# AdrienCorenflos/aux-ssm-samplers

Hardware: AMD Instinct MI355X
Metric: Gibbs sweeps/sec (aux-Kalman, parallel-in-time scan) (higher is better)
Workload: dtype f64; 1 GPU; C2: linear-Gaussian SSM T=65536 d=4 p=8, aux-Kalman sweep, parallel scan; chains_per_gpu=256, parallelism=chains x1 (independent, no collective)

## Files before the change

aux_ssm_samplers_amd/csrc/api.hip:

```cpp
#include <cstdarg>
#include <cstdlib>
#include <cstring>

#include "ctx.h"
#include "rng.h"

namespace ax {

static thread_local std::string g_err;
void set_error(const char* fmt, ...) {
    char buf[1024];
    va_list ap;
    va_start(ap, fmt);
    vsnprintf(buf, sizeof buf, fmt, ap);
    va_end(ap);
    g_err = buf;
}

int ws_reserve(auxssm_ctx* h, size_t bytes) {
    h->ws_off = 0;
    if (bytes <= h->ws_bytes) return AUXSSM_OK;
    if (h->ws) {
        AX_HIP(hipStreamSynchronize(h->stream));
        AX_HIP(hipFree(h->ws));
// ... 620 lines not shown
    SampleArgs sa;
    sa.d = kd;
    sa.dx = D;
    sa.Fs = cv(model->Fs); sa.Qs = cv(model->Qs); sa.bs = cv(model->bs);
    sa.ms = msA; sa.Ps = PsA; sa.eps = epsA; sa.xs = xpA; sa.elem = nullptr;
    sa.lay = ScanLayout{1, 1, 1, 1, cm, C};
    sa.ps_shared = shared_mode ? 1 : 0;
    sa.ps_packed = ps_pack ? 1 : 0;
    if (gen) sa.eps_gen = 1, sa.gen_k0 = keys[2], sa.gen_k1 = keys[3];
    rc = se->sample(h, sa, parallel);
    if (rc) return rc;
    h->ws_off = mark;

    {
        SweepLogpdfArgs la;
        la.d = kd;
        la.dx = D; la.po = PO;
        la.m0 = cv(model->m0); la.P0 = cv(model->P0); la.Fs = cv(model->Fs); la.Qs = cv(model->Qs); la.bs = cv(model->bs);
        la.Hs = cv(model->Hs); la.Rs = cv(model->Rs); la.cs = cv(model->cs); la.ys = cv(*yobs);
        la.x = xA; la.xp = xpA; la.u = uA; la.delta = delta; la.nan_policy = nan_policy;
        la.u_fly = aux_fly ? 1 : 0; la.eps_aux = epsauxA; la.shd = sqrt(0.5 * delta); la.dptr = dptr;
        rc = sl->run(h, la, sums);
        if (rc) return rc;
        h->ws_off = mark;
    }
    const Acc* jp_prop = sums; const Acc* jp_rev = sums + C; const Acc* lt_prop = sums + 2 * C; const Acc* lt_rev = sums + 3 * C; const Acc* corr = sums + 4 * C;
    hipLaunchKernelGGL((k_accept<R>), dim3((C + 127) / 128), dim3(128), 0, h->stream, C, jp_prop, jp_rev, (const R*)ell, (const R*)ell, lt_prop, lt_rev,
                       corr, (const R*)u_acc, accepted, (R*)logs);
    if ((rc = launch_select<R>(h, C, T, D, (const int32_t*)accepted, xpA, xA, cm))) return rc;
    AX_HIP(hipGetLastError());
    return AUXSSM_OK;
}

template <typename R>
__global__ void k_fs_concat0(int C, int D, int PO, const R* __restrict__ xa, const R* __restrict__ xb, const int32_t* __restrict__ sel, const R* __restrict__ eps0, R shd,
                             const double* dptr, Arr yobs, R* __restrict__ u, R* __restrict__ ysc0) {
    if (dptr) shd = (R)dptr[1];
    const int P = D + PO;
    const int g = blockIdx.x * blockDim.x + threadIdx.x;
    if (g >= C * P) return;
    const int c = g % C, k = g / C;
    if (k < D) {
        const R* x = (sel && sel[c]) ? xb : xa;
        const R v = x[(long long)k * C + c] + shd * eps0[(long long)k * C + c];
        u[(long long)k * C + c] = v;
        ysc0[(long long)k * C + c] = v;
    } else {
        ysc0[(long long)k * C + c] = at<R>(yobs, 0, 0, 0)[k - D];
    }
}
template <typename R> __global__ void __launch_bounds__(256) k_fs_resolve(int C, const int32_t* __restrict__ sel, const R* __restrict__ xb, R* __restrict__ xa) {
    const int c = blockIdx.y * 256 + threadIdx.x;
    if (c >= C) return;
    const long long off = (long long)blockIdx.x * C + c;
    if (sel[c]) xa[off] = xb[off];
}
template <typename R>
__global__ void __launch_bounds__(256) k_fs_stats(int C, const int32_t* __restrict__ accepted, const int32_t* __restrict__ sel, const R* __restrict__ xa, const R* __restrict__ xb,
                                                   R* __restrict__ sq_jump, R* __restrict__ mean, R* __restrict__ sq_mean, long long iter) {
    const int c = blockIdx.y * 256 + threadIdx.x;
    if (c >= C) return;
    const long long off = (long long)blockIdx.x * C + c;
    const int s = sel[c], acc = accepted[c];
    const R xn = (s ? xb : xa)[off];
    const R xo = acc ? (s ? xa : xb)[off] : xn;
    const R it = (R)iter, dj = xn - xo;
    sq_jump[off] = fold_mean<R>(it, sq_jump[off], dj * dj);
    mean[off] = fold_mean<R>(it, mean[off], xn);
    sq_mean[off] = fold_mean<R>(it, sq_mean[off], xn * xn);
}
static const char* fused_refusal(const auxssm_ctx* h, const auxssm_dims* dims, const auxssm_lgssm* model, int parallel, int layout) {
    const int C = dims->C, T = dims->T, D = dims->dx, PO = dims->dy;
    if (layout != AUXSSM_LAYOUT_CHAIN_MINOR) return "the fused sweep takes the chain-minor layout";
    if (D > MAX_D || PO < 1 || PO > 4) return "the fused sweep is instantiated for dx <= 4, 1 <= dy <= 4";
    if (!parallel) return "the fused sweep is the parallel-in-time one";
    if (!h->share_model) return "AUXSSM_OPT_SHARE_MODEL is off";
    if (!(model->Fs.sc == 0 && model->Qs.sc == 0 && model->bs.sc == 0 && model->P0.sc == 0 && model->m0.sc == 0))
        return "the fused sweep needs chain-shared model parameters (chain stride 0)";
    if (C < 2 || (C % 2) != 0) return "the fused sweep pairs chains for its in-kernel draws: the chain count must be even";
    if (T < 64) return "the fused sweep needs T >= 64";
    return nullptr;
}
template <typename R>
static int sweep_lg_concat_fused(auxssm_ctx* h, int dtype, const auxssm_dims* dims, const auxssm_lgssm* model, const auxssm_arr* yobs, double delta, const double* dptr,
                                 const uint32_t* keys, int nan_policy, void* x, void* x_alt, int32_t* sel, void* u_acc, int32_t* accepted, void* logs) {
    const int C = dims->C, T = dims->T, D = dims->dx, PO = dims->dy, P = D + PO;
    const SweepLogpdfEntry* sl = sweep_logpdf_entry(dtype, D, PO);
    if (!sl || !sl->fused) {
        set_error("(dx=%d, dy=%d) has no fused sweep in this build", D, PO);
        return AUXSSM_ERR_UNSUPPORTED;
    }
    const KDims kd{C, T, 1};
    const size_t sR = sizeof(R), CT = (size_t)C * T;
    size_t need = 0;
    auto add = [&](size_t b) { need += b + 256; };
    add(CT * D * sR);
    add(CT * D * sR);
    add((size_t)T * (P * D + P * P + P + D * D) * sR);
    add(1024);
    add((size_t)C * (P + 3 * D) * sR + 1024);
    add(sl->fused_ws(h, kd));
    int rc = ws_reserve(h, need);
    if (rc) return rc;
    R* u = (R*)ws_take(h, CT * D * sR);
    R* inc = (R*)ws_take(h, CT * D * sR);
    R* ysc0 = (R*)ws_take(h, (size_t)C * P * sR);
    R* m0p = (R*)ws_take(h, (size_t)C * D * sR);
    R* eps0a = (R*)ws_take(h, (size_t)C * D * sR);
    R* eps0s = (R*)ws_take(h, (size_t)C * D * sR);
    if (!u || !inc || !ysc0 || !m0p || !eps0a || !eps0s) return AUXSSM_ERR_NOMEM;
    bool overlap = h->overlap_model_stage != 0 && !dptr;
    struct SweepEnd {
        auxssm_ctx* h;
        ~SweepEnd() { side_sweep_end(h); }
    } sweep_end{h};
    if (overlap) {
        const size_t need_side = sl->fused_ws(h, kd) + (size_t)(T + 64) * sR * ((size_t)P * D + (size_t)P * P + P + (size_t)D * D) + (4u << 20) +
                                 (size_t)(T + 2) * sR * (3 * (size_t)D * D + 2 * D + (size_t)PO * D + (size_t)PO * PO + 2 * PO);
        if ((rc = side_open(h, need_side))) return rc;
        overlap = h->side.open;
    }
    R *Hc, *Rc, *cc, *Ps;
    const bool tinv = model->Hs.st == 0 && model->Rs.st == 0 && model->cs.st == 0;
    const int Tm = tinv ? 1 : T;
    const int* memo = nullptr;
    struct MemoGuard {
        auxssm_ctx* h;
        int p = -1;
        bool ok = false;
        ~MemoGuard() { if (p >= 0 && !ok) h->side.memo_use[p] = -1; }
    } memo_guard{h};
    if (overlap) {
        SideScope sc(h);
        auxssm_ctx::SideStage& sd = h->side;
        const int p = sd.parity;
        MemoDesc md{};
        const auxssm_arr* srcs[9] = {&model->m0, &model->P0, &model->Fs, &model->Qs, &model->bs, &model->Hs, &model->Rs, &model->cs, yobs};
        const int recs[9] = {D, D * D, D * D, D * D, D, PO * D, PO * PO, PO, PO};
        const int nts[9] = {1, 1, T - 1, T - 1, T - 1, T, T, T, T};
        md.n = 9;
        md.off[0] = 0;
        bool plain = true;
        for (int q = 0; q < 9; ++q) {
// ... 10 lines not shown
            std::vector<unsigned char> key;
            auto put = [&](const void* v, size_t nb) { key.insert(key.end(), (const unsigned char*)v, (const unsigned char*)v + nb); };
            const int hdr[8] = {(int)sR, C, T, D, PO, nan_policy, 0, 0};
            put(hdr, sizeof(hdr));
            put(&delta, sizeof(delta));
            for (int q = 0; q < 9; ++q) put(srcs[q], sizeof(auxssm_arr));
            const bool chain_ok = sd.memo_use[p] == sd.uses[p] - 1 && sd.memo_key[p] == key;
            const unsigned gmemo = (unsigned)std::min<long long>(1024, (md.off[9] + 255) / 256);
            if (chain_ok) {
                hipLaunchKernelGGL(k_memo_set, dim3(1), dim3(1), 0, h->stream, rebuild, 0);
                hipLaunchKernelGGL((k_memo_check<R>), dim3(gmemo), dim3(256), 0, h->stream, md, (const R*)snap, rebuild);
            } else {
                hipLaunchKernelGGL(k_memo_set, dim3(1), dim3(1), 0, h->stream, rebuild, 1);
            }
            hipLaunchKernelGGL((k_memo_snap<R>), dim3(gmemo), dim3(256), 0, h->stream, md, snap, (const int*)rebuild);
            sd.memo_key[p] = std::move(key);
            sd.memo_use[p] = sd.uses[p];
            memo_guard.p = p;
            memo = rebuild;
        }
    }
    {
        SideScope sc(h);
        Hc = (R*)ws_take(h, (size_t)T * P * D * sR);
        Rc = (R*)ws_take(h, (size_t)T * P * P * sR);
        cc = (R*)ws_take(h, (size_t)T * P * sR);
        Ps = (R*)ws_take(h, (size_t)T * D * D * sR);
        if (!Hc || !Rc || !cc || !Ps) return AUXSSM_ERR_NOMEM;
        ProfScope ps(h, AUXSSM_K_FACTORY);
        const long long n1 = (long long)Tm * (P * D + P * P + P);
        hipLaunchKernelGGL((k_concat_model<R>), dim3((unsigned)((n1 + 255) / 256)), dim3(256), 0, h->stream, Tm, D, PO, cv(model->Hs), cv(model->Rs), cv(model->cs),
                           (R)(0.5 * delta), dptr, Hc, Rc, cc, memo);
    }
    launch_rng_sweep<R>(h, keys, (long long)D * C, C, eps0a, eps0s, u_acc);
    hipLaunchKernelGGL((k_fs_concat0<R>), dim3((unsigned)((C * P + 255) / 256)), dim3(256), 0, h->stream, C, D, PO, (const R*)x, (const R*)x_alt, (const int32_t*)sel,
                       (const R*)eps0a, (R)sqrt(0.5 * delta), dptr, cv(*yobs), u, ysc0);
    FusedHost f{};
    auxssm_lgssm gc = *model;
    gc.Hs = auxssm_arr{Hc, 0, tinv ? 0 : (int64_t)P * D, 0};
    gc.Rs = auxssm_arr{Rc, 0, tinv ? 0 : (int64_t)P * P, 0};
    gc.cs = auxssm_arr{cc, 0, tinv ? 0 : (int64_t)P, 0};
    const auxssm_arr ysc_dummy{ysc0, (int64_t)P, (int64_t)P, 0};
    auxssm_dims dc = *dims;
    dc.dy = P;
    dc.B = 1;
    fill_filter_args(f.fa, &dc, &gc, &ysc_dummy, m0p, Ps);
    const KDims k1{C, 1, 1};
    f.fa.ys = cm_arr(ysc0, k1, P);
    f.fa.ms = cm_arr(m0p, k1, D);
    f.fa.Ps = Arr{Ps, 0, (long long)D * D, 0, 1};
    f.fa.lay.cm = 1;
    f.fa.pblk = D;
    f.fa.aux_on = 1;
    f.fa.aux_yobs = cv(*yobs);
    f.fa.aux_shd = sqrt(0.5 * delta);
    f.fa.dptr = dptr;
    f.sa.d = kd;
    f.sa.dx = D;
    f.sa.Fs = cv(model->Fs); f.sa.Qs = cv(model->Qs); f.sa.bs = cv(model->bs);
    f.sa.Ps = f.fa.Ps;
    f.sa.ps_shared = 1;
    f.sa.elem = nullptr;
    f.sa.lay = ScanLayout{1, 1, 1, 1, 1, C};
    SweepLogpdfArgs& la = f.la;
    la.d = kd;
    la.dx = D; la.po = PO;
    la.m0 = cv(model->m0); la.P0 = cv(model->P0); la.Fs = cv(model->Fs); la.Qs = cv(model->Qs); la.bs = cv(model->bs);
    la.Hs = cv(model->Hs); la.Rs = cv(model->Rs); la.cs = cv(model->cs); la.ys = cv(*yobs);
    la.x = cm_arr(x, kd, D); la.xp = cm_arr(x_alt, kd, D); la.u = cm_arr(u, kd, D);
// ... 1108 lines not shown
```

aux_ssm_samplers_amd/csrc/ctx.h:

```cpp
#pragma once
#include <hip/hip_runtime.h>
#include <cstdio>
#include <string>
#include <vector>

#include "../../include/auxssm.h"
#include "kalman_bodies.h"

namespace ax {

void set_error(const char* fmt, ...);
void fk_modules_release(auxssm_ctx* h);

#define AX_HIP(expr)                                                                         \
    do {                                                                                     \
        hipError_t _e = (expr);                                                              \
        if (_e != hipSuccess) {                                                              \
            ax::set_error("%s failed: %s (%s:%d)", #expr, hipGetErrorString(_e), __FILE__, __LINE__); \
            return AUXSSM_ERR_HIP;                                                           \
        }                                                                                    \
    } while (0)

#define AX_NEED_H(h)                          \
    do {                                      \
// ... 134 lines not shown
};
constexpr int SCAN_WAVES_MAX = 4;
ScanPlan plan_scan(const auxssm_ctx* h, int S, int n, int parallel, int waves = 1);
struct AffPlan {
    int E, nchunk;
};
AffPlan plan_aff(const auxssm_ctx* h, int S, int N, int parallel, int waves = 8);

typedef int (*filter_fn)(auxssm_ctx*, const FilterArgs&, int parallel, void* ell_out );
typedef int (*sample_fn)(auxssm_ctx*, const SampleArgs&, int parallel);
typedef int (*logpdf_fn)(auxssm_ctx*, const LogpdfArgs&, void* out );
typedef size_t (*filter_ws_fn)(const auxssm_ctx*, const KDims&, int parallel);
typedef size_t (*sample_ws_fn)(const auxssm_ctx*, const KDims&, int parallel);
typedef size_t (*logpdf_ws_fn)(const auxssm_ctx*, const KDims&);

struct KalmanEntry {
    filter_fn filter;
    filter_ws_fn filter_ws;
    logpdf_fn logpdf;
    logpdf_ws_fn logpdf_ws;
};
typedef int (*sweep_logpdf_fn)(auxssm_ctx*, const SweepLogpdfArgs&, void* out );
typedef size_t (*sweep_logpdf_ws_fn)(const auxssm_ctx*, const KDims&);
struct FusedHost {
    FilterArgs fa;
    SampleArgs sa;
    SweepLogpdfArgs la;
    const void* xa;
    void* xb;
    int32_t* sel;
    void* u;
    void* inc;
    const uint32_t* keys;
    const void* eps0s;
    const void* u_acc;
    int32_t* accepted;
    void* logs;
    const int* memo = nullptr;
};
typedef int (*fused_fn)(auxssm_ctx*, FusedHost&);
typedef size_t (*fused_ws_fn)(const auxssm_ctx*, const KDims&);
struct SweepLogpdfEntry {
    sweep_logpdf_fn run;
    sweep_logpdf_ws_fn ws;
    sweep_logpdf_fn lorenz = nullptr;
    fused_fn fused = nullptr;
    fused_ws_fn fused_ws = nullptr;
    sweep_logpdf_fn wide_shared = nullptr;
};
typedef int (*sv_logpdf_fn)(auxssm_ctx*, const SvLogpdfArgs&, void* out );
typedef size_t (*sv_logpdf_ws_fn)(const auxssm_ctx*, const KDims&);
struct SampleEntry {
    sample_fn sample;
    sample_ws_fn sample_ws;
    sv_logpdf_fn sv_logpdf = nullptr;
    sv_logpdf_ws_fn sv_logpdf_ws = nullptr;
};

constexpr int MAX_D = 4;
constexpr int MAX_P = 8;

const KalmanEntry* kalman_entry(int dtype, int D, int P);
const SampleEntry* sample_entry(int dtype, int D);
const SweepLogpdfEntry* sweep_logpdf_entry(int dtype, int D, int PO);

const KalmanEntry* wide_kalman_entry(int dtype);
const SampleEntry* wide_sample_entry(int dtype);
const SweepLogpdfEntry* wide_sweep_logpdf_entry(int dtype);
// ... 8 lines not shown
```

aux_ssm_samplers_amd/csrc/fused_shared.h:

```cpp
#pragma once

struct FusedArgs {
    int C, T, E, nchunk;
    const void* xa;
    void* xb;
    const int32_t* sel;
    void* u;
    void* inc;
    const void* gain;
    const void* samp;
    const void* logt;
    const void* gpre;
    const void* m0p;
    void* agg_f; void* pre_f; void* agg_s; void* pre_s;
    Acc* pa;
    Acc* pe;
    void* pell;
    const Acc* clog;
    unsigned ka0, ka1, ks0, ks1;
    const void* eps0s;
    double delta, shd;
    const double* dptr;
    int nan_policy;
    const int* memo;
// ... 51 lines not shown
#pragma unroll
        for (int k = 0; k < D * D; ++k) G[k] = row[TS::oG + k];
        mm<R, D, D, D>(M, G, o);
#pragma unroll
        for (int k = 0; k < D * D; ++k) M[k] = o[k];
    }
#pragma unroll
    for (int k = 0; k < D * D; ++k) cprod[(long long)(a.nchunk - 1 - ch) * D * D + k] = M[k];
}

template <typename R, int D> __global__ void __launch_bounds__(TB_CM) k_fs_psi(FusedArgs a, const R* __restrict__ gpre, const R* __restrict__ fpre, R* __restrict__ ntab,
                                                                              R* __restrict__ psi) {
    if (memo_skip(a)) return;
    using TS = SampShared<R, D>;
    const int ch = blockIdx.x * TB_CM + threadIdx.x;
    if (ch >= a.nchunk) return;
    const int t0 = ch * a.E, tb = min(a.T, t0 + a.E);
    R Ps[D * D];
#pragma unroll
    for (int k = 0; k < D * D; ++k) Ps[k] = 0;
    for (int t = t0; t < tb; ++t) {
        const R* row = (const R*)a.samp + (long long)t * TS::NPAD;
        R M1[D * D], Ph[D * D], Gp[D * D], Nt[D * D], o[D * D];
#pragma unroll
        for (int k = 0; k < D * D; ++k) M1[k] = row[TS::oM + k], Ph[k] = fpre[(long long)t * D * D + k], Gp[k] = gpre[(long long)t * D * D + k];
        mm<R, D, D, D>(M1, Ph, Nt);
        mm<R, D, D, D>(Gp, Nt, o);
#pragma unroll
        for (int k = 0; k < D * D; ++k) ntab[(long long)t * D * D + k] = Nt[k], Ps[k] += o[k];
    }
#pragma unroll
    for (int k = 0; k < D * D; ++k) psi[(long long)ch * D * D + k] = Ps[k];
}
template <typename R, int D> __global__ void __launch_bounds__(256) k_fs_esfix(int C, int nchunk, const R* __restrict__ psi, const R* __restrict__ pre_f, R* __restrict__ agg_s) {
    const long long g = (long long)blockIdx.x * 256 + threadIdx.x;
    if (g >= (long long)C * nchunk) return;
    const int c = (int)(g / nchunk), ch = (int)(g % nchunk);
    if (ch == 0) return;
    R m[D], e[D], Ps[D * D];
    ldv<R, D>(pre_f + ((long long)c * nchunk + ch) * SampPre<R, D>::NPAD, m);
    R* q = agg_s + ((long long)c * nchunk + (nchunk - 1 - ch)) * SampPre<R, D>::NPAD;
    ldv<R, D>(q, e);
#pragma unroll
    for (int k = 0; k < D * D; ++k) Ps[k] = psi[(long long)ch * D * D + k];
#pragma unroll
    for (int i = 0; i < D; ++i) {
        R v = e[i];
#pragma unroll
        for (int k = 0; k < D; ++k) v += Ps[i * D + k] * m[k];
        e[i] = v;
    }
    stv<R, D>(q, e);
}

template <typename R, int D, int PO> struct FsRows {
    static constexpr int P = D + PO;
    using TL = LogShared<R, D, PO>;
    static constexpr int VEC = 16 / sizeof(R);
    static constexpr int pad(int n) { return (n + VEC - 1) / VEC * VEC; }
    static constexpr int cM = 0, cKc = D * D, cK = cKc + D, cM1 = cK + D * D, cGb = cM1 + D * D, cL = cGb + D, cGp = cL + symsize(D), cLg = cGp + D * D,
                         NC = pad(cLg + TL::N);
    static constexpr int eG = 0, eN = D * D, eL = 2 * D * D, NE = pad(eL + TL::N);
};
struct FsSrc { int tab, off; };
template <typename R, int D, int PO> __device__ __forceinline__ FsSrc fs_src_c(int k) {
    constexpr int P = D + PO;
    using F = FsRows<R, D, PO>; using TG = GainRow<R, D, P>; using TS = SampShared<R, D>; using TL = LogShared<R, D, PO>;
    if (k < F::cKc) return {0, TG::oM + k};
    if (k < F::cK) return {0, TG::oKc + (k - F::cKc)};
    if (k < F::cM1) { const int q = k - F::cK; return {0, TG::oK + (q / D) * P + (q % D)}; }
    if (k < F::cGb) return {1, TS::oM + (k - F::cM1)};
    if (k < F::cL) return {1, TS::oGb + (k - F::cGb)};
    if (k < F::cGp) {
        const int q = k - F::cL;
        int i = 0;
        while (lidx(i + 1, 0) <= q) ++i;
        return {1, TS::oL + i * D + (q - lidx(i, 0))};
    }
    if (k < F::cLg) return {3, k - F::cGp};
    if (k < F::cLg + TL::N) return {2, k - F::cLg};
    return {-1, 0};
}
template <typename R, int D, int PO> __device__ __forceinline__ FsSrc fs_src_e(int k) {
    using F = FsRows<R, D, PO>; using TS = SampShared<R, D>; using TL = LogShared<R, D, PO>;
    if (k < F::eN) return {1, TS::oG + k};
// ... 387 lines not shown
        R inc[D], ut[D], xp[D];
#pragma unroll
        for (int k = 0; k < D; ++k) inc[k] = incn[k], ut[k] = utn[k];
        if (t > t0) {
            const int tn = PK ? t - 1 : opaque_uniform(t - 1);
#pragma unroll
            for (int k = 0; k < D; ++k) incn[k] = ip[((long long)tn * D + k) * C], utn[k] = up[((long long)tn * D + k) * C];
        }
#pragma unroll
        for (int i = 0; i < D; ++i) {
            R v = inc[i];
#pragma unroll
            for (int k = 0; k < D; ++k) v += row[F::eN + i * D + k] * mst[k];
#pragma unroll
            for (int k = 0; k < D; ++k) v += row[F::eG + i * D + k] * h[k];
            xp[i] = v;
            xw[((long long)tu * D + i) * C] = v;
        }
        if (tu + 1 < a.T) {
            R w[3];
            if (fs_wave_any(fs_terms_fast<R, D, PO>(row + F::eL, h, xp, uq, inv_delta, cst, w))) fs_terms<R, D, PO>(a, row + F::eL, h, xp, uq, inv_delta, cst, w);
            v0 += (Acc)w[0];
            v1 += (Acc)w[1];
            v2 += (Acc)w[2];
        }
#pragma unroll
        for (int k = 0; k < D; ++k) h[k] = xp[k], uq[k] = ut[k];
    }
    a.pe[((long long)0 * C + c) * a.nchunk + ch] = v0;
    a.pe[((long long)1 * C + c) * a.nchunk + ch] = v1;
    a.pe[((long long)2 * C + c) * a.nchunk + ch] = v2;
}

template <typename R, int D, int PO> __global__ void __launch_bounds__(TB_ELEM) k_fs_head(SweepLogpdfArgs la, const void* xa, const void* xb, const int32_t* sel, R* __restrict__ head5) {
    resolve_step(la);
    const int c = blockIdx.x * TB_ELEM + threadIdx.x;
    if (c >= la.d.C) return;
    const bool sw = sel && sel[c];
    la.x.ptr = sw ? xb : xa;
    la.xp.ptr = sw ? xa : xb;
    R h5[5];
    body_sweep_logpdf_head<R, D, PO>(la, c, h5);
#pragma unroll
    for (int k = 0; k < 5; ++k) head5[(long long)k * la.d.C + c] = h5[k];
}

template <typename R> __global__ void __launch_bounds__(TB_ELEM) k_fs_accept(FusedArgs a, const R* __restrict__ head5, const R* __restrict__ ell0,
                                                                            const R* __restrict__ u_acc, int32_t* __restrict__ accepted, R* __restrict__ logs,
                                                                            int32_t* __restrict__ sel) {
    __shared__ Acc sh[TB_ELEM];
    const int c = blockIdx.x;
    const long long C = a.C;
    Acc tot[7] = {0, 0, 0, 0, 0, 0, 0};
    const R* pl = (const R*)a.pell + (long long)c * a.nchunk;
    for (int j = threadIdx.x; j < a.nchunk; j += TB_ELEM) {
#pragma unroll
        for (int k = 0; k < 3; ++k) tot[k] += a.pa[((long long)k * C + c) * a.nchunk + j], tot[3 + k] += a.pe[((long long)k * C + c) * a.nchunk + j];
        tot[6] += (Acc)pl[j];
    }
#pragma unroll
    for (int k = 0; k < 7; ++k) tot[k] = block_sum<Acc, TB_ELEM>(tot[k], sh);
    if (threadIdx.x != 0) return;
    (void)ell0;
    const Acc jp_prop = tot[3] + (Acc)head5[0 * C + c], jp_rev = tot[0] + (Acc)head5[1 * C + c];
    const Acc ell = jp_prop - (tot[6] - *a.clog);
    const Acc lt_prop = tot[4] + (Acc)head5[2 * C + c], lt_rev = tot[1] + (Acc)head5[3 * C + c];
    const Acc corr = (tot[5] - tot[2]) + (Acc)head5[4 * C + c];
    const Acc lp_prop = jp_prop - ell, lp_rev = jp_rev - ell;
    Acc la = lt_prop - lt_rev;
    la += lp_rev - lp_prop;
    la -= corr;
    const Acc alpha = exp_(la != la ? la : min_(la, (Acc)0));
    const int acc = ((Acc)u_acc[c] < alpha) ? 1 : 0;
    accepted[c] = acc;
    if (sel) sel[c] ^= acc;
    if (logs) {
        logs[c * 5 + 0] = (R)la;
        logs[c * 5 + 1] = (R)lp_prop;
        logs[c * 5 + 2] = (R)lp_rev;
        logs[c * 5 + 3] = (R)lt_prop;
        logs[c * 5 + 4] = (R)lt_rev;
    }
}

inline int fs_pack(int C, int* cp_out) {
    int cp = 2;
    while (cp < C) cp <<= 1;
    *cp_out = cp;
    constexpr int lanes = 256;
    if (cp > lanes / 2) return 1;
    const int pack = lanes / cp;
    constexpr int cap = 8;
    return pack > cap ? cap : pack;
}
inline int fs_chunk_len(const auxssm_ctx* h, int C, int T) {
    constexpr int waves = 10;
    const long long stiles = (C + TB_CM - 1) / TB_CM;
    long long want = (long long)h->num_cu * 4 * waves / stiles;
    if (want < 1) want = 1;
    long long E = (T + want - 1) / want;
    if (E < 16) E = 16;
    if (E > 32) E = 32;
    if (C >= 1024) E = 64;
    else if (C >= 96) E = 32;
    if (E > T) E = T > 2 ? T : 2;
    return (int)E;
}
template <typename R, int D, int PO> size_t fused_ws(const auxssm_ctx* h, const KDims& d) {
    constexpr int P = D + PO;
    const int E = fs_chunk_len(h, d.C, d.T), nchunk = (d.T + E - 1) / E;
    size_t b = 0;
    b += (size_t)d.C * nchunk * (4 * SampPre<R, D>::NPAD * sizeof(R) + 6 * sizeof(Acc) + sizeof(R)) + 16 * 256;
    b += (size_t)d.C * (5 + 1 + D) * sizeof(R) + 4 * 256;
    b += filter_ws<R, D, P>(h, KDims{1, d.T, 1}, 1);
    b += (size_t)d.T * (SampShared<R, D>::NPAD + LogShared<R, D, PO>::NPAD + (size_t)D * D) * sizeof(R) + (size_t)2 * nchunk * D * D * sizeof(R) + 10 * 256 + ((size_t)d.T / 256 + 2) * sizeof(Acc);
    b += (size_t)d.T * (FsRows<R, D, PO>::NC + FsRows<R, D, PO>::NE + 2 * (size_t)D * D) * sizeof(R) + (size_t)nchunk * D * D * sizeof(R) + 8 * 256;
    return b;
}
template <typename R, int D, int PO> int run_fused_shared(auxssm_ctx* h, FusedHost& f) {
    constexpr int P = D + PO;
    const int C = f.fa.d.C, T = f.fa.d.T, n = T - 1;
    FusedArgs a{};
    a.C = C; a.T = T;
    a.E = fs_chunk_len(h, C, T);
    a.nchunk = (T + a.E - 1) / a.E;
    a.pack = fs_pack(C, &a.cp);
    {
        using FR = FsRows<R, D, PO>;
        constexpr int NMAX = FR::NC > FR::NE ? FR::NC : FR::NE;
        while (a.pack > 1 && (size_t)a.pack * fs_pk_block<R, NMAX>(a.E) * sizeof(R) + FsNormTabSel<R>::BYTES > (size_t)128 * 1024) a.pack >>= 1;
    }
    a.xa = f.xa; a.xb = f.xb; a.sel = f.sel; a.u = f.u; a.inc = f.inc;
    a.ka0 = f.keys[0]; a.ka1 = f.keys[1]; a.ks0 = f.keys[2]; a.ks1 = f.keys[3];
    a.eps0s = f.eps0s;
    a.delta = f.la.delta; a.shd = f.la.shd; a.dptr = f.la.dptr; a.nan_policy = f.la.nan_policy;
    a.memo = f.memo;
    f.fa.memo = f.sa.memo = f.la.memo = f.memo;
    R *cprod_f, *cprod_s, *rows_c, *rows_e, *psi;
    {
        {
            const int rc = build_gain_table<R, D, P>(h, f.fa);
            if (rc) return rc;
        }
        SideScope side(h);
        f.sa.tab = ws_take(h, (size_t)T * SampShared<R, D>::NPAD * sizeof(R));
        f.la.tab = ws_take(h, (size_t)n * LogShared<R, D, PO>::NPAD * sizeof(R));
        R* gpre = (R*)ws_take(h, (size_t)T * D * D * sizeof(R));
        cprod_f = (R*)ws_take(h, (size_t)a.nchunk * D * D * sizeof(R));
        cprod_s = (R*)ws_take(h, (size_t)a.nchunk * D * D * sizeof(R));
        rows_c = (R*)ws_take(h, (size_t)T * FsRows<R, D, PO>::NC * sizeof(R));
        rows_e = (R*)ws_take(h, (size_t)T * FsRows<R, D, PO>::NE * sizeof(R));
        R* fpre = (R*)ws_take(h, (size_t)T * D * D * sizeof(R));
        R* ntab = (R*)ws_take(h, (size_t)T * D * D * sizeof(R));
        psi = (R*)ws_take(h, (size_t)a.nchunk * D * D * sizeof(R));
        const int nclb = (T + 255) / 256;
        Acc* clog = (Acc*)ws_take(h, 256 + (size_t)nclb * sizeof(Acc));
        if (!f.sa.tab || !f.la.tab || !gpre || !cprod_f || !cprod_s || !rows_c || !rows_e || !fpre || !ntab || !psi || !clog) return AUXSSM_ERR_NOMEM;
        a.clog = clog;
        a.gain = f.fa.tab; a.samp = f.sa.tab; a.logt = f.la.tab; a.gpre = gpre;
        {
            ProfScope ps(h, AUXSSM_K_SAMPLE_INIT);
            hipLaunchKernelGGL((k_sample_shared_tab<R, D>), dim3((T + TB_ELEM - 1) / TB_ELEM), dim3(TB_ELEM), 0, h->stream, f.sa);
            hipLaunchKernelGGL((k_fs_clog_part<R, D>), dim3(nclb), dim3(256), 0, h->stream, T, (const R*)f.sa.tab, clog + 32, f.memo);
            hipLaunchKernelGGL((k_fs_clog_sum<D>), dim3(1), dim3(256), 0, h->stream, T, nclb, (const Acc*)(clog + 32), clog, f.memo);
            hipLaunchKernelGGL((k_sweep_logpdf_tab<R, D, PO>), dim3((n + TB_ELEM - 1) / TB_ELEM), dim3(TB_ELEM), 0, h->stream, f.la);
            hipLaunchKernelGGL((k_fs_fprod<R, D, P>), dim3((a.nchunk + TB_CM - 1) / TB_CM), dim3(TB_CM), 0, h->stream, a, cprod_f, fpre);
            hipLaunchKernelGGL((k_fs_gpre<R, D>), dim3((a.nchunk + TB_CM - 1) / TB_CM), dim3(TB_CM), 0, h->stream, a, gpre, cprod_s);
            hipLaunchKernelGGL((k_fs_psi<R, D>), dim3((a.nchunk + TB_CM - 1) / TB_CM), dim3(TB_CM), 0, h->stream, a, (const R*)gpre, (const R*)fpre, ntab, psi);
            {
                using F = FsRows<R, D, PO>;
                const long long nmax = (long long)T * (F::NC > F::NE ? F::NC : F::NE);
                hipLaunchKernelGGL((k_fs_rows<R, D, PO>), dim3((unsigned)((nmax + 255) / 256), 2), dim3(256), 0, h->stream, a, (const R*)ntab, rows_c, rows_e);
            }
        }
    }
    {
        const int rc = side_close(h);
        if (rc) return rc;
    }
    a.memo = nullptr;
    f.fa.memo = f.sa.memo = f.la.memo = nullptr;
    const size_t npre = (size_t)C * a.nchunk * SampPre<R, D>::NPAD * sizeof(R);
    a.agg_f = ws_take(h, npre); a.pre_f = ws_take(h, npre); a.agg_s = ws_take(h, npre); a.pre_s = ws_take(h, npre);
    a.pa = (Acc*)ws_take(h, (size_t)3 * C * a.nchunk * sizeof(Acc));
    a.pe = (Acc*)ws_take(h, (size_t)3 * C * a.nchunk * sizeof(Acc));
    a.pell = ws_take(h, (size_t)C * a.nchunk * sizeof(R));
    R* head5 = (R*)ws_take(h, (size_t)5 * C * sizeof(R));
    f.fa.ell0 = ws_take(h, (size_t)C * sizeof(R));
    if (!a.agg_f || !a.pre_f || !a.agg_s || !a.pre_s || !a.pa || !a.pe || !a.pell || !head5 || !f.fa.ell0) return AUXSSM_ERR_NOMEM;
    a.m0p = f.fa.ms.ptr;
    f.fa.t0_keep_ps = 1;
    hipLaunchKernelGGL((k_filter_t0<R, D, P>), dim3((C + TB_ELEM - 1) / TB_ELEM), dim3(TB_ELEM), 0, h->stream, f.fa);
    using F = FsRows<R, D, PO>;
    const int TBF = C >= 256 ? 256 : (C + 63) / 64 * 64;
    const unsigned grid = (unsigned)a.nchunk * (unsigned)((C + TBF - 1) / TBF);
    const unsigned grid_pk = (unsigned)((a.nchunk + a.pack - 1) / a.pack);
    const size_t lds = (size_t)TB_AGGS * SampElem<R, D>::NPAD * sizeof(R);
    if (a.pack > 1) {
        const size_t lds_ac = (size_t)a.pack * fs_pk_block<R, F::NC>(a.E) * sizeof(R) + FsNormTabSel<R>::BYTES;
        if (lds_ac > 64 * 1024) AX_HIP(hipFuncSetAttribute((const void*)k_fs_ac<R, D, PO, true>, hipFuncAttributeMaxDynamicSharedMemorySize, (int)lds_ac));
        ProfScope ps(h, AUXSSM_K_FILTER_SCAN);
        hipLaunchKernelGGL((k_fs_ac<R, D, PO, true>), dim3(grid_pk), dim3(a.pack * a.cp), lds_ac, h->stream, a, (const R*)rows_c);
    } else {
        const size_t lds_ac = (size_t)a.E * F::NC * sizeof(R) + FsNormTabSel<R>::BYTES;
        if (lds_ac > 64 * 1024) AX_HIP(hipFuncSetAttribute((const void*)k_fs_ac<R, D, PO>, hipFuncAttributeMaxDynamicSharedMemorySize, (int)lds_ac));
        ProfScope ps(h, AUXSSM_K_FILTER_SCAN);
        hipLaunchKernelGGL((k_fs_ac<R, D, PO>), dim3(grid), dim3(TBF), lds_ac, h->stream, a, (const R*)rows_c);
    }
    {
        ProfScope ps(h, AUXSSM_K_SAMPLE_SCAN);
        hipLaunchKernelGGL((k_aff_aggs<R, D>), dim3(C), dim3(TB_AGGS), lds, h->stream, ScanBufs{a.agg_f, a.pre_f}, (const R*)cprod_f, a.nchunk);
        hipLaunchKernelGGL((k_fs_esfix<R, D>), dim3((unsigned)(((long long)C * a.nchunk + 255) / 256)), dim3(256), 0, h->stream, C, a.nchunk, (const R*)psi, (const R*)a.pre_f,
                           (R*)a.agg_s);
        hipLaunchKernelGGL((k_aff_aggs<R, D>), dim3(C), dim3(TB_AGGS), lds, h->stream, ScanBufs{a.agg_s, a.pre_s}, (const R*)cprod_s, a.nchunk);
    }
    {
        ProfScope ps(h, AUXSSM_K_LOGPDF);
        if (a.pack > 1) {
            const size_t lds_e = (size_t)a.pack * fs_pk_block<R, F::NE>(a.E) * sizeof(R);
            if (lds_e > 64 * 1024) AX_HIP(hipFuncSetAttribute((const void*)k_fs_e<R, D, PO, true>, hipFuncAttributeMaxDynamicSharedMemorySize, (int)lds_e));
            hipLaunchKernelGGL((k_fs_e<R, D, PO, true>), dim3(grid_pk), dim3(a.pack * a.cp), lds_e, h->stream, a, (const R*)rows_e);
        } else
            hipLaunchKernelGGL((k_fs_e<R, D, PO>), dim3(grid), dim3(TBF), (size_t)a.E * F::NE * sizeof(R), h->stream, a, (const R*)rows_e);
    }
    {
        ProfScope ps(h, AUXSSM_K_SELECT);
        hipLaunchKernelGGL((k_fs_head<R, D, PO>), dim3((C + TB_ELEM - 1) / TB_ELEM), dim3(TB_ELEM), 0, h->stream, f.la, f.xa, (const void*)f.xb, (const int32_t*)f.sel, head5);
        hipLaunchKernelGGL((k_fs_accept<R>), dim3(C), dim3(TB_ELEM), 0, h->stream, a, (const R*)head5, (const R*)f.fa.ell0, (const R*)f.u_acc, f.accepted,
                           (R*)f.logs, f.sel);
    }
    AX_HIP(hipGetLastError());
    return AUXSSM_OK;
}
```

aux_ssm_samplers_amd/csrc/kernels.hip.h:

```cpp
#pragma once
#include <algorithm>
#include <type_traits>
#include <cstdlib>

#include "ctx.h"
#include "affine_shared.h"

namespace ax {

constexpr int TB_ELEM = 128;
constexpr int TB_SCAN = 64;
constexpr int TB_AGGS = 256;

template <typename R, int TB> __device__ __forceinline__ R block_sum(R v, R* sh) {
    const int tid = threadIdx.x;
    sh[tid] = v;
    __syncthreads();
#pragma unroll
    for (int off = TB / 2; off > 0; off >>= 1) {
        if (tid < off) sh[tid] += sh[tid + off];
        __syncthreads();
    }
    const R r = sh[0];
    __syncthreads();
    return r;
}

template <typename R> struct WaveIO {
    R* lds;
    int lane;
    int nvalid;
    template <typename R2, int N> __device__ __forceinline__ void fetch(const R2* lane_ptr, long long stride, long long se, bool valid, R2* buf) const {
        static_assert(sizeof(R2) == sizeof(R), "one real type per kernel");
        if (se == 1 && (stride == N || stride == -N)) {
            const R2* p0 = stride < 0 ? lane_ptr + (long long)(lane - (nvalid - 1)) * N : lane_ptr - (long long)lane * N;
            const int total = nvalid * N;
#pragma unroll
            for (int j = 0; j < N; ++j) {
                const int q = j * 64 + lane;
// ... 1386 lines not shown
```

Measured before the change: 281,700 sweeps/s.

## Fuse sweep prologue, mid scans, and head/accept kernels; precompute shared scan level products

Merges the RNG, concat0 and filter-t0 kernels into one prologue kernel that draws its normals inline. Replaces the two k_aff_aggs scans and the esfix pass with a single per-chain kernel. That kernel reuses chain-independent per-level matrix products, precomputed once by a small k_fs_glev kernel, so each chain only does matrix-vector work. The head logpdf computation moves into the accept kernel on an extra wavefront. The aim is to cut kernel launches, global round-trips and redundant matrix-matrix products in the scan, at the cost of more complex kernels and a serial head computation inside the accept block.

```diff
diff --git a/aux_ssm_samplers_amd/csrc/api.hip b/aux_ssm_samplers_amd/csrc/api.hip
--- a/aux_ssm_samplers_amd/csrc/api.hip
+++ b/aux_ssm_samplers_amd/csrc/api.hip
@@ -676,23 +676,6 @@
     return AUXSSM_OK;
 }
 
-template <typename R>
-__global__ void k_fs_concat0(int C, int D, int PO, const R* __restrict__ xa, const R* __restrict__ xb, const int32_t* __restrict__ sel, const R* __restrict__ eps0, R shd,
-                             const double* dptr, Arr yobs, R* __restrict__ u, R* __restrict__ ysc0) {
-    if (dptr) shd = (R)dptr[1];
-    const int P = D + PO;
-    const int g = blockIdx.x * blockDim.x + threadIdx.x;
-    if (g >= C * P) return;
-    const int c = g % C, k = g / C;
-    if (k < D) {
-        const R* x = (sel && sel[c]) ? xb : xa;
-        const R v = x[(long long)k * C + c] + shd * eps0[(long long)k * C + c];
-        u[(long long)k * C + c] = v;
-        ysc0[(long long)k * C + c] = v;
-    } else {
-        ysc0[(long long)k * C + c] = at<R>(yobs, 0, 0, 0)[k - D];
-    }
-}
 template <typename R> __global__ void __launch_bounds__(256) k_fs_resolve(int C, const int32_t* __restrict__ sel, const R* __restrict__ xb, R* __restrict__ xa) {
     const int c = blockIdx.y * 256 + threadIdx.x;
     if (c >= C) return;
@@ -742,7 +725,7 @@
     add(CT * D * sR);
     add((size_t)T * (P * D + P * P + P + D * D) * sR);
     add(1024);
-    add((size_t)C * (P + 3 * D) * sR + 1024);
+    add((size_t)C * (P + 2 * D) * sR + 1024);
     add(sl->fused_ws(h, kd));
     int rc = ws_reserve(h, need);
     if (rc) return rc;
@@ -750,9 +733,8 @@
     R* inc = (R*)ws_take(h, CT * D * sR);
     R* ysc0 = (R*)ws_take(h, (size_t)C * P * sR);
     R* m0p = (R*)ws_take(h, (size_t)C * D * sR);
-    R* eps0a = (R*)ws_take(h, (size_t)C * D * sR);
     R* eps0s = (R*)ws_take(h, (size_t)C * D * sR);
-    if (!u || !inc || !ysc0 || !m0p || !eps0a || !eps0s) return AUXSSM_ERR_NOMEM;
+    if (!u || !inc || !ysc0 || !m0p || !eps0s) return AUXSSM_ERR_NOMEM;
     bool overlap = h->overlap_model_stage != 0 && !dptr;
     struct SweepEnd {
         auxssm_ctx* h;
@@ -829,9 +811,6 @@
         hipLaunchKernelGGL((k_concat_model<R>), dim3((unsigned)((n1 + 255) / 256)), dim3(256), 0, h->stream, Tm, D, PO, cv(model->Hs), cv(model->Rs), cv(model->cs),
                            (R)(0.5 * delta), dptr, Hc, Rc, cc, memo);
     }
-    launch_rng_sweep<R>(h, keys, (long long)D * C, C, eps0a, eps0s, u_acc);
-    hipLaunchKernelGGL((k_fs_concat0<R>), dim3((unsigned)((C * P + 255) / 256)), dim3(256), 0, h->stream, C, D, PO, (const R*)x, (const R*)x_alt, (const int32_t*)sel,
-                       (const R*)eps0a, (R)sqrt(0.5 * delta), dptr, cv(*yobs), u, ysc0);
     FusedHost f{};
     auxssm_lgssm gc = *model;
     gc.Hs = auxssm_arr{Hc, 0, tinv ? 0 : (int64_t)P * D, 0};
diff --git a/aux_ssm_samplers_amd/csrc/ctx.h b/aux_ssm_samplers_amd/csrc/ctx.h
--- a/aux_ssm_samplers_amd/csrc/ctx.h
+++ b/aux_ssm_samplers_amd/csrc/ctx.h
@@ -190,8 +190,8 @@
     void* u;
     void* inc;
     const uint32_t* keys;
-    const void* eps0s;
-    const void* u_acc;
+    void* eps0s;
+    void* u_acc;
     int32_t* accepted;
     void* logs;
     const int* memo = nullptr;
diff --git a/aux_ssm_samplers_amd/csrc/fused_scan.h b/aux_ssm_samplers_amd/csrc/fused_scan.h
--- /dev/null
+++ b/aux_ssm_samplers_amd/csrc/fused_scan.h
@@ -0,0 +1,141 @@
+#pragma once
+#include "smallmat.h"
+
+namespace ax {
+
+constexpr int FSC_LANES = 256;
+constexpr int FSC_LEVELS = 8;
+constexpr int FSC_BATCH = 8;
+
+template <typename R, int D> struct FscRec {
+    static constexpr int VEC = 16 / sizeof(R);
+    static constexpr int NPAD = (D + VEC - 1) / VEC * VEC;
+};
+
+template <typename R, int D> AX_HD void fsc_ldm(const R* p, R* out) {
+    if constexpr ((D * D * sizeof(R)) % 16 == 0) ldv<R, D * D>(p, out);
+    else ld<R, D * D>(p, out);
+}
+template <typename R, int D> AX_HD void fsc_stm(R* p, const R* v) {
+    if constexpr ((D * D * sizeof(R)) % 16 == 0) stv<R, D * D>(p, v);
+    else st<R, D * D>(p, v);
+}
+
+AX_HD void fsc_range(int nchunk, int tid, int& j0, int& j1) {
+    const int E2 = (nchunk + FSC_LANES - 1) / FSC_LANES;
+    j0 = tid * E2 < nchunk ? tid * E2 : nchunk;
+    j1 = j0 + E2 < nchunk ? j0 + E2 : nchunk;
+}
+
+template <typename R, int D> AX_HD void fsc_g_fold(const R* cprod, int j0, int j1, R* G) {
+#pragma unroll
+    for (int k = 0; k < D * D; ++k) G[k] = (k / D == k % D) ? (R)1 : (R)0;
+    if (j0 < j1) fsc_ldm<R, D>(cprod + (long long)j0 * D * D, G);
+    for (int j = j0 + 1; j < j1; ++j) {
+        R c[D * D], o[D * D];
+        fsc_ldm<R, D>(cprod + (long long)j * D * D, c);
+        mm<R, D, D, D>(c, G, o);
+#pragma unroll
+        for (int k = 0; k < D * D; ++k) G[k] = o[k];
+    }
+}
+template <typename R, int D> AX_HD void fsc_g_level(const R* Gleft, R* G) {
+    R o[D * D];
+    mm<R, D, D, D>(G, Gleft, o);
+#pragma unroll
+    for (int k = 0; k < D * D; ++k) G[k] = o[k];
+}
+template <int D> AX_HD long long fsc_glev_off(int lev, int tid) { return ((long long)lev * FSC_LANES + tid) * D * D; }
+
+template <typename R, int D> AX_HD void fsc_e_step(const R* G, const R* p, const R* e, R* o) {
+    R t[D];
+    mv<R, D, D>(G, p, t);
+#pragma unroll
+    for (int i = 0; i < D; ++i) o[i] = t[i] + e[i];
+}
+template <typename R, int D> AX_HD void fsc_e_fold(const R* cprod, const R* agg, int j0, int j1, R* acc) {
+    constexpr int NP = FscRec<R, D>::NPAD;
+#pragma unroll
+    for (int i = 0; i < D; ++i) acc[i] = 0;
+    for (int jb = j0; jb < j1; jb += FSC_BATCH) {
+        R ev[FSC_BATCH][D];
+#pragma unroll
+        for (int q = 0; q < FSC_BATCH; ++q)
+            if (jb + q < j1) ldv<R, D>(agg + (long long)(jb + q) * NP, ev[q]);
+#pragma unroll
+        for (int q = 0; q < FSC_BATCH; ++q) {
+            if (jb + q >= j1) continue;
+            if (jb + q == j0) {
+#pragma unroll
+                for (int i = 0; i < D; ++i) acc[i] = ev[q][i];
+            } else {
+                R c[D * D], o[D];
+                fsc_ldm<R, D>(cprod + (long long)(jb + q) * D * D, c);
+                fsc_e_step<R, D>(c, acc, ev[q], o);
+#pragma unroll
+                for (int i = 0; i < D; ++i) acc[i] = o[i];
+            }
+        }
+    }
+}
+template <typename R, int D> AX_HD void fsc_e_level(const R* Glev, const R* left, R* acc) {
+    R o[D];
+    fsc_e_step<R, D>(Glev, left, acc, o);
+#pragma unroll
+    for (int i = 0; i < D; ++i) acc[i] = o[i];
+}
+template <typename R, int D> AX_HD void fsc_e_walk(const R* cprod, const R* agg, R* pre, int j0, int j1, const R* ex) {
+    constexpr int NP = FscRec<R, D>::NPAD;
+    R p[D];
+#pragma unroll
+    for (int i = 0; i < D; ++i) p[i] = ex[i];
+    for (int jb = j0; jb < j1; jb += FSC_BATCH) {
+        R ev[FSC_BATCH][D];
+#pragma unroll
+        for (int q = 0; q < FSC_BATCH; ++q)
+            if (jb + q + 1 < j1) ldv<R, D>(agg + (long long)(jb + q) * NP, ev[q]);
+#pragma unroll
+        for (int q = 0; q < FSC_BATCH; ++q) {
+            if (jb + q >= j1) continue;
+            stv<R, D>(pre + (long long)(jb + q) * NP, p);
+            if (jb + q + 1 < j1) {
+                R c[D * D], o[D];
+                fsc_ldm<R, D>(cprod + (long long)(jb + q) * D * D, c);
+                fsc_e_step<R, D>(c, p, ev[q], o);
+#pragma unroll
+                for (int i = 0; i < D; ++i) p[i] = o[i];
+            }
+        }
+    }
+}
+template <typename R, int D> AX_HD void fsc_s_complete(const R* psi, const R* pre_f, R* agg_s, int nchunk, int j0, int j1) {
+    constexpr int NP = FscRec<R, D>::NPAD;
+    for (int jb = j0; jb < j1; jb += FSC_BATCH) {
+        R ev[FSC_BATCH][D], mv_[FSC_BATCH][D];
+#pragma unroll
+        for (int q = 0; q < FSC_BATCH; ++q) {
+            const int ch = nchunk - 1 - (jb + q);
+            if (jb + q < j1 && ch > 0) {
+                ldv<R, D>(agg_s + (long long)(jb + q) * NP, ev[q]);
+                ldv<R, D>(pre_f + (long long)ch * NP, mv_[q]);
+            }
+        }
+#pragma unroll
+        for (int q = 0; q < FSC_BATCH; ++q) {
+            const int ch = nchunk - 1 - (jb + q);
+            if (jb + q >= j1 || ch <= 0) continue;
+            R Ps[D * D];
+            fsc_ldm<R, D>(psi + (long long)ch * D * D, Ps);
+#pragma unroll
+            for (int i = 0; i < D; ++i) {
+                R v = ev[q][i];
+#pragma unroll
+                for (int k = 0; k < D; ++k) v += Ps[i * D + k] * mv_[q][k];
+                ev[q][i] = v;
+            }
+            stv<R, D>(agg_s + (long long)(jb + q) * NP, ev[q]);
+        }
+    }
+}
+
+}
diff --git a/aux_ssm_samplers_amd/csrc/fused_shared.h b/aux_ssm_samplers_amd/csrc/fused_shared.h
--- a/aux_ssm_samplers_amd/csrc/fused_shared.h
+++ b/aux_ssm_samplers_amd/csrc/fused_shared.h
@@ -107,25 +107,70 @@
 #pragma unroll
     for (int k = 0; k < D * D; ++k) psi[(long long)ch * D * D + k] = Ps[k];
 }
-template <typename R, int D> __global__ void __launch_bounds__(256) k_fs_esfix(int C, int nchunk, const R* __restrict__ psi, const R* __restrict__ pre_f, R* __restrict__ agg_s) {
-    const long long g = (long long)blockIdx.x * 256 + threadIdx.x;
-    if (g >= (long long)C * nchunk) return;
-    const int c = (int)(g / nchunk), ch = (int)(g % nchunk);
-    if (ch == 0) return;
-    R m[D], e[D], Ps[D * D];
-    ldv<R, D>(pre_f + ((long long)c * nchunk + ch) * SampPre<R, D>::NPAD, m);
-    R* q = agg_s + ((long long)c * nchunk + (nchunk - 1 - ch)) * SampPre<R, D>::NPAD;
-    ldv<R, D>(q, e);
-#pragma unroll
-    for (int k = 0; k < D * D; ++k) Ps[k] = psi[(long long)ch * D * D + k];
-#pragma unroll
-    for (int i = 0; i < D; ++i) {
-        R v = e[i];
-#pragma unroll
-        for (int k = 0; k < D; ++k) v += Ps[i * D + k] * m[k];
-        e[i] = v;
-    }
-    stv<R, D>(q, e);
+static_assert(FSC_LANES == TB_AGGS, "fused_scan.h scans with k_aff_aggs' lanes");
+template <typename R, int D> __global__ void __launch_bounds__(TB_AGGS) k_fs_glev(FusedArgs a, const R* __restrict__ cprod_f, const R* __restrict__ cprod_s, R* __restrict__ glev_f,
+                                                                                 R* __restrict__ glev_s) {
+    if (memo_skip(a)) return;
+    __shared__ __attribute__((aligned(16))) R sh[TB_AGGS * D * D];
+    const R* cprod = blockIdx.x ? cprod_s : cprod_f;
+    R* glev = blockIdx.x ? glev_s : glev_f;
+    const int tid = threadIdx.x;
+    int j0, j1;
+    fsc_range(a.nchunk, tid, j0, j1);
+    R G[D * D];
+    fsc_g_fold<R, D>(cprod, j0, j1, G);
+    for (int lev = 0, off = 1; lev < FSC_LEVELS; ++lev, off <<= 1) {
+        fsc_stm<R, D>(glev + fsc_glev_off<D>(lev, tid), G);
+        st<R, D * D>(sh + tid * D * D, G);
+        __syncthreads();
+        R left[D * D];
+        if (tid >= off) ld<R, D * D>(sh + (tid - off) * D * D, left);
+        __syncthreads();
+        if (tid >= off) fsc_g_level<R, D>(left, G);
+    }
+}
+template <typename R, int D> __device__ __forceinline__ void fs_scan_chain(const R* __restrict__ cprod, const R* __restrict__ glev, const R* agg, R* pre, int nchunk, R* sh) {
+    constexpr int NP = FscRec<R, D>::NPAD;
+    const int tid = threadIdx.x;
+    int j0, j1;
+    fsc_range(nchunk, tid, j0, j1);
+    R acc[D];
+    fsc_e_fold<R, D>(cprod, agg, j0, j1, acc);
+    for (int lev = 0, off = 1; lev < FSC_LEVELS; ++lev, off <<= 1) {
+        R* buf = sh + (lev & 1) * TB_AGGS * NP;
+        stv<R, D>(buf + tid * NP, acc);
+        R G[D * D];
+        if (tid >= off) fsc_ldm<R, D>(glev + fsc_glev_off<D>(lev, tid), G);
+        __syncthreads();
+        if (tid >= off) {
+            R left[D];
+            ldv<R, D>(buf + (tid - off) * NP, left);
+            fsc_e_level<R, D>(G, left, acc);
+        }
+    }
+    static_assert(FSC_LEVELS % 2 == 0, "the totals go to buffer 0, last read two barriers ago");
+    stv<R, D>(sh + tid * NP, acc);
+    __syncthreads();
+    R ex[D];
+#pragma unroll
+    for (int k = 0; k < D; ++k) ex[k] = 0;
+    if (tid > 0) ldv<R, D>(sh + (tid - 1) * NP, ex);
+    fsc_e_walk<R, D>(cprod, agg, pre, j0, j1, ex);
+}
+template <typename R, int D> __global__ void __launch_bounds__(TB_AGGS) k_fs_mid(FusedArgs a, const R* __restrict__ cprod_f, const R* __restrict__ glev_f, const R* __restrict__ cprod_s,
+                                                                                const R* __restrict__ glev_s, const R* __restrict__ psi) {
+    constexpr int NP = FscRec<R, D>::NPAD;
+    static_assert(NP == SampPre<R, D>::NPAD, "record stride of the aggregates");
+    __shared__ __attribute__((aligned(16))) R sh[2 * TB_AGGS * NP];
+    const long long rec = (long long)blockIdx.x * a.nchunk * NP;
+    R* pre_f = (R*)a.pre_f + rec;
+    R* agg_s = (R*)a.agg_s + rec;
+    fs_scan_chain<R, D>(cprod_f, glev_f, (const R*)a.agg_f + rec, pre_f, a.nchunk, sh);
+    __syncthreads();
+    int j0, j1;
+    fsc_range(a.nchunk, threadIdx.x, j0, j1);
+    fsc_s_complete<R, D>(psi, pre_f, agg_s, a.nchunk, j0, j1);
+    fs_scan_chain<R, D>(cprod_s, glev_s, agg_s, (R*)a.pre_s + rec, a.nchunk, sh);
 }
 
 template <typename R, int D, int PO> struct FsRows {
@@ -579,28 +624,27 @@
     a.pe[((long long)2 * C + c) * a.nchunk + ch] = v2;
 }
 
-template <typename R, int D, int PO> __global__ void __launch_bounds__(TB_ELEM) k_fs_head(SweepLogpdfArgs la, const void* xa, const void* xb, const int32_t* sel, R* __restrict__ head5) {
-    resolve_step(la);
-    const int c = blockIdx.x * TB_ELEM + threadIdx.x;
-    if (c >= la.d.C) return;
-    const bool sw = sel && sel[c];
-    la.x.ptr = sw ? xb : xa;
-    la.xp.ptr = sw ? xa : xb;
-    R h5[5];
-    body_sweep_logpdf_head<R, D, PO>(la, c, h5);
-#pragma unroll
-    for (int k = 0; k < 5; ++k) head5[(long long)k * la.d.C + c] = h5[k];
-}
-
-template <typename R> __global__ void __launch_bounds__(TB_ELEM) k_fs_accept(FusedArgs a, const R* __restrict__ head5, const R* __restrict__ ell0,
-                                                                            const R* __restrict__ u_acc, int32_t* __restrict__ accepted, R* __restrict__ logs,
-                                                                            int32_t* __restrict__ sel) {
-    __shared__ Acc sh[TB_ELEM];
+constexpr int FS_TB_ACCEPT = TB_ELEM + 64;
+template <typename R, int D, int PO>
+__global__ void __launch_bounds__(FS_TB_ACCEPT) k_fs_accept(FusedArgs a, SweepLogpdfArgs lg, const R* __restrict__ ell0, const R* __restrict__ u_acc, int32_t* __restrict__ accepted,
+                                                            R* __restrict__ logs, int32_t* __restrict__ sel) {
+    __shared__ Acc sh[FS_TB_ACCEPT];
+    __shared__ R head5[5];
     const int c = blockIdx.x;
+    if (threadIdx.x == TB_ELEM) {
+        resolve_step(lg);
+        const bool sw = sel && sel[c];
+        lg.x.ptr = sw ? a.xb : a.xa;
+        lg.xp.ptr = sw ? a.xa : a.xb;
+        R h5[5];
+        body_sweep_logpdf_head<R, D, PO>(lg, c, h5);
+#pragma unroll
+        for (int k = 0; k < 5; ++k) head5[k] = h5[k];
+    }
     const long long C = a.C;
     Acc tot[7] = {0, 0, 0, 0, 0, 0, 0};
     const R* pl = (const R*)a.pell + (long long)c * a.nchunk;
-    for (int j = threadIdx.x; j < a.nchunk; j += TB_ELEM) {
+    for (int j = threadIdx.x < TB_ELEM ? threadIdx.x : a.nchunk; j < a.nchunk; j += TB_ELEM) {
 #pragma unroll
         for (int k = 0; k < 3; ++k) tot[k] += a.pa[((long long)k * C + c) * a.nchunk + j], tot[3 + k] += a.pe[((long long)k * C + c) * a.nchunk + j];
         tot[6] += (Acc)pl[j];
@@ -609,10 +653,10 @@
     for (int k = 0; k < 7; ++k) tot[k] = block_sum<Acc, TB_ELEM>(tot[k], sh);
     if (threadIdx.x != 0) return;
     (void)ell0;
-    const Acc jp_prop = tot[3] + (Acc)head5[0 * C + c], jp_rev = tot[0] + (Acc)head5[1 * C + c];
+    const Acc jp_prop = tot[3] + (Acc)head5[0], jp_rev = tot[0] + (Acc)head5[1];
     const Acc ell = jp_prop - (tot[6] - *a.clog);
-    const Acc lt_prop = tot[4] + (Acc)head5[2 * C + c], lt_rev = tot[1] + (Acc)head5[3 * C + c];
-    const Acc corr = (tot[5] - tot[2]) + (Acc)head5[4 * C + c];
+    const Acc lt_prop = tot[4] + (Acc)head5[2], lt_rev = tot[1] + (Acc)head5[3];
+    const Acc corr = (tot[5] - tot[2]) + (Acc)head5[4];
     const Acc lp_prop = jp_prop - ell, lp_rev = jp_rev - ell;
     Acc la = lt_prop - lt_rev;
     la += lp_rev - lp_prop;
@@ -630,6 +674,30 @@
     }
 }
 
+template <typename R, int D, int PO>
+__global__ void __launch_bounds__(TB_ELEM) k_fs_pro(FusedArgs a, FilterArgs fa, unsigned kc0, unsigned kc1, R* eps0s, R* u_acc, R* ysc0) {
+    constexpr int P = D + PO;
+    fs_resolve(a);
+    const int c = blockIdx.x * TB_ELEM + threadIdx.x;
+    if (c >= a.C) return;
+    const long long C = a.C;
+    const R* x = (const R*)((a.sel && a.sel[c]) ? (const void*)a.xb : a.xa);
+    const R shd = (R)a.shd;
+#pragma unroll
+    for (int k = 0; k < D; ++k) {
+        const R ea = stream_normal<R>(a.ka0, a.ka1, 0, (unsigned long long)(k * C + c));
+        eps0s[k * C + c] = stream_normal<R>(a.ks0, a.ks1, 0, (unsigned long long)(k * C + c));
+        const R v = x[k * C + c] + shd * ea;
+        ((R*)a.u)[k * C + c] = v;
+        ysc0[k * C + c] = v;
+    }
+    const R* y0 = at<R>(fa.aux_yobs, 0, 0, 0);
+#pragma unroll
+    for (int k = 0; k < PO; ++k) ysc0[(D + k) * C + c] = y0[k];
+    u_acc[c] = stream_uniform<R>(kc0, kc1, 0, (unsigned long long)c);
+    body_filter_t0<R, D, P>(fa, c);
+}
+
 inline int fs_pack(int C, int* cp_out) {
     int cp = 2;
     while (cp < C) cp <<= 1;
@@ -658,10 +726,11 @@
     const int E = fs_chunk_len(h, d.C, d.T), nchunk = (d.T + E - 1) / E;
     size_t b = 0;
     b += (size_t)d.C * nchunk * (4 * SampPre<R, D>::NPAD * sizeof(R) + 6 * sizeof(Acc) + sizeof(R)) + 16 * 256;
-    b += (size_t)d.C * (5 + 1 + D) * sizeof(R) + 4 * 256;
+    b += (size_t)d.C * (1 + D) * sizeof(R) + 4 * 256;
     b += filter_ws<R, D, P>(h, KDims{1, d.T, 1}, 1);
     b += (size_t)d.T * (SampShared<R, D>::NPAD + LogShared<R, D, PO>::NPAD + (size_t)D * D) * sizeof(R) + (size_t)2 * nchunk * D * D * sizeof(R) + 10 * 256 + ((size_t)d.T / 256 + 2) * sizeof(Acc);
     b += (size_t)d.T * (FsRows<R, D, PO>::NC + FsRows<R, D, PO>::NE + 2 * (size_t)D * D) * sizeof(R) + (size_t)nchunk * D * D * sizeof(R) + 8 * 256;
+    b += (size_t)2 * FSC_LEVELS * TB_AGGS * D * D * sizeof(R) + 2 * 256;
     return b;
 }
 template <typename R, int D, int PO> int run_fused_shared(auxssm_ctx* h, FusedHost& f) {
@@ -683,7 +752,7 @@
     a.delta = f.la.delta; a.shd = f.la.shd; a.dptr = f.la.dptr; a.nan_policy = f.la.nan_policy;
     a.memo = f.memo;
     f.fa.memo = f.sa.memo = f.la.memo = f.memo;
-    R *cprod_f, *cprod_s, *rows_c, *rows_e, *psi;
+    R *cprod_f, *cprod_s, *rows_c, *rows_e, *psi, *glev_f, *glev_s;
     {
         {
             const int rc = build_gain_table<R, D, P>(h, f.fa);
@@ -700,9 +769,12 @@
         R* fpre = (R*)ws_take(h, (size_t)T * D * D * sizeof(R));
         R* ntab = (R*)ws_take(h, (size_t)T * D * D * sizeof(R));
         psi = (R*)ws_take(h, (size_t)a.nchunk * D * D * sizeof(R));
+        const size_t nglev = (size_t)FSC_LEVELS * TB_AGGS * D * D * sizeof(R);
+        glev_f = (R*)ws_take(h, nglev);
+        glev_s = (R*)ws_take(h, nglev);
         const int nclb = (T + 255) / 256;
         Acc* clog = (Acc*)ws_take(h, 256 + (size_t)nclb * sizeof(Acc));
-        if (!f.sa.tab || !f.la.tab || !gpre || !cprod_f || !cprod_s || !rows_c || !rows_e || !fpre || !ntab || !psi || !clog) return AUXSSM_ERR_NOMEM;
+        if (!f.sa.tab || !f.la.tab || !gpre || !cprod_f || !cprod_s || !rows_c || !rows_e || !fpre || !ntab || !psi || !glev_f || !glev_s || !clog) return AUXSSM_ERR_NOMEM;
         a.clog = clog;
         a.gain = f.fa.tab; a.samp = f.sa.tab; a.logt = f.la.tab; a.gpre = gpre;
         {
@@ -714,6 +786,7 @@
             hipLaunchKernelGGL((k_fs_fprod<R, D, P>), dim3((a.nchunk + TB_CM - 1) / TB_CM), dim3(TB_CM), 0, h->stream, a, cprod_f, fpre);
             hipLaunchKernelGGL((k_fs_gpre<R, D>), dim3((a.nchunk + TB_CM - 1) / TB_CM), dim3(TB_CM), 0, h->stream, a, gpre, cprod_s);
             hipLaunchKernelGGL((k_fs_psi<R, D>), dim3((a.nchunk + TB_CM - 1) / TB_CM), dim3(TB_CM), 0, h->stream, a, (const R*)gpre, (const R*)fpre, ntab, psi);
+            hipLaunchKernelGGL((k_fs_glev<R, D>), dim3(2), dim3(TB_AGGS), 0, h->stream, a, (const R*)cprod_f, (const R*)cprod_s, glev_f, glev_s);
             {
                 using F = FsRows<R, D, PO>;
                 const long long nmax = (long long)T * (F::NC > F::NE ? F::NC : F::NE);
@@ -732,17 +805,19 @@
     a.pa = (Acc*)ws_take(h, (size_t)3 * C * a.nchunk * sizeof(Acc));
     a.pe = (Acc*)ws_take(h, (size_t)3 * C * a.nchunk * sizeof(Acc));
     a.pell = ws_take(h, (size_t)C * a.nchunk * sizeof(R));
-    R* head5 = (R*)ws_take(h, (size_t)5 * C * sizeof(R));
     f.fa.ell0 = ws_take(h, (size_t)C * sizeof(R));
-    if (!a.agg_f || !a.pre_f || !a.agg_s || !a.pre_s || !a.pa || !a.pe || !a.pell || !head5 || !f.fa.ell0) return AUXSSM_ERR_NOMEM;
+    if (!a.agg_f || !a.pre_f || !a.agg_s || !a.pre_s || !a.pa || !a.pe || !a.pell || !f.fa.ell0) return AUXSSM_ERR_NOMEM;
     a.m0p = f.fa.ms.ptr;
     f.fa.t0_keep_ps = 1;
-    hipLaunchKernelGGL((k_filter_t0<R, D, P>), dim3((C + TB_ELEM - 1) / TB_ELEM), dim3(TB_ELEM), 0, h->stream, f.fa);
+    {
+        ProfScope ps(h, AUXSSM_K_RNG);
+        hipLaunchKernelGGL((k_fs_pro<R, D, PO>), dim3((C + TB_ELEM - 1) / TB_ELEM), dim3(TB_ELEM), 0, h->stream, a, f.fa, f.keys[4], f.keys[5], (R*)f.eps0s, (R*)f.u_acc,
+                           (R*)const_cast<void*>(f.fa.ys.ptr));
+    }
     using F = FsRows<R, D, PO>;
     const int TBF = C >= 256 ? 256 : (C + 63) / 64 * 64;
     const unsigned grid = (unsigned)a.nchunk * (unsigned)((C + TBF - 1) / TBF);
     const unsigned grid_pk = (unsigned)((a.nchunk + a.pack - 1) / a.pack);
-    const size_t lds = (size_t)TB_AGGS * SampElem<R, D>::NPAD * sizeof(R);
     if (a.pack > 1) {
         const size_t lds_ac = (size_t)a.pack * fs_pk_block<R, F::NC>(a.E) * sizeof(R) + FsNormTabSel<R>::BYTES;
         if (lds_ac > 64 * 1024) AX_HIP(hipFuncSetAttribute((const void*)k_fs_ac<R, D, PO, true>, hipFuncAttributeMaxDynamicSharedMemorySize, (int)lds_ac));
@@ -756,10 +831,7 @@
     }
     {
         ProfScope ps(h, AUXSSM_K_SAMPLE_SCAN);
-        hipLaunchKernelGGL((k_aff_aggs<R, D>), dim3(C), dim3(TB_AGGS), lds, h->stream, ScanBufs{a.agg_f, a.pre_f}, (const R*)cprod_f, a.nchunk);
-        hipLaunchKernelGGL((k_fs_esfix<R, D>), dim3((unsigned)(((long long)C * a.nchunk + 255) / 256)), dim3(256), 0, h->stream, C, a.nchunk, (const R*)psi, (const R*)a.pre_f,
-                           (R*)a.agg_s);
-        hipLaunchKernelGGL((k_aff_aggs<R, D>), dim3(C), dim3(TB_AGGS), lds, h->stream, ScanBufs{a.agg_s, a.pre_s}, (const R*)cprod_s, a.nchunk);
+        hipLaunchKernelGGL((k_fs_mid<R, D>), dim3(C), dim3(TB_AGGS), 0, h->stream, a, (const R*)cprod_f, (const R*)glev_f, (const R*)cprod_s, (const R*)glev_s, (const R*)psi);
     }
     {
         ProfScope ps(h, AUXSSM_K_LOGPDF);
@@ -772,9 +844,7 @@
     }
     {
         ProfScope ps(h, AUXSSM_K_SELECT);
-        hipLaunchKernelGGL((k_fs_head<R, D, PO>), dim3((C + TB_ELEM - 1) / TB_ELEM), dim3(TB_ELEM), 0, h->stream, f.la, f.xa, (const void*)f.xb, (const int32_t*)f.sel, head5);
-        hipLaunchKernelGGL((k_fs_accept<R>), dim3(C), dim3(TB_ELEM), 0, h->stream, a, (const R*)head5, (const R*)f.fa.ell0, (const R*)f.u_acc, f.accepted,
-                           (R*)f.logs, f.sel);
+        hipLaunchKernelGGL((k_fs_accept<R, D, PO>), dim3(C), dim3(FS_TB_ACCEPT), 0, h->stream, a, f.la, (const R*)f.fa.ell0, (const R*)f.u_acc, f.accepted, (R*)f.logs, f.sel);
     }
     AX_HIP(hipGetLastError());
     return AUXSSM_OK;
diff --git a/aux_ssm_samplers_amd/csrc/kernels.hip.h b/aux_ssm_samplers_amd/csrc/kernels.hip.h
--- a/aux_ssm_samplers_amd/csrc/kernels.hip.h
+++ b/aux_ssm_samplers_amd/csrc/kernels.hip.h
@@ -5,6 +5,7 @@
 
 #include "ctx.h"
 #include "affine_shared.h"
+#include "fused_scan.h"
 
 namespace ax {
 
```

Measured after the change: 282,000 sweeps/s (median of 4 runs). About the same (+0.1%).
